# manish-pra/sampling-gpmpc

Hardware: AMD Instinct MI355X
Metric: sampled trajectory-steps/sec (Ns*H per wall second) (higher is better)
Workload: dtype f64; 1 GPU; BASELINE configs[1]: params_pendulum1D_samples, sequential re-conditioned rollout (mode R, value+gradient labels T=3), Ns=1024 per GPU, H=30; Ns_per_gpu=1024, H=30, Ns_total=1024, device=AMD Radeon Graphics (gfx950:sramecc+:xnack-), cus=256

## Files before the change

sampling_gpmpc_amd/csrc/build.py:

```python
#!/usr/bin/env python3
import hashlib
import json
import os
import subprocess
import sys
from concurrent.futures import ThreadPoolExecutor

HERE = os.path.dirname(os.path.abspath(__file__))
REPO = os.path.dirname(os.path.dirname(HERE))
SOURCES = ["capi.hip", "rollout.hip", "rollout_fast.hip", "rollout_tiles.hip", "rollout_one.hip", "rollout_indep.hip", "joint.hip",
           "joint_mfma.hip", "joint_chol.hip", "assemble.hip", "base_samples.hip", "hull.hip",
           "hull_query.hip", "sup_dev.hip", "mll.hip", "moments.hip", "moments_grad.hip", "tube_qp.hip", "tube_rows.hip", "pathwise.hip",
           "pathwise_stats.hip", "pathwise_grad.hip", "pathwise_cand.hip", "robust_tube.hip", "robust_tube_grad.hip", "lipschitz.hip", "contraction.hip",
           "optimistic.hip"]
HEADERS = ["gpmpc_device.hpp", "gpmpc_host.hpp", "rollout_args.hpp", "rollout_plan.hpp", "joint_args.hpp", "joint_eigh.hpp", "joint_plan.hpp", "hull_geom.hpp", "min_index.hpp", "base_stream.hpp", "moments_step.hpp", "pathwise_step.hpp", "robust_step.hpp", "contraction_math.hpp",
           "rollout_one_gen.inc", "rollout_tiles_mfma.inc", "joint_mfma_gen.inc",
           os.path.join(REPO, "include", "gpmpc_hip.h")]
GENERATED = {"rollout_one_gen.inc": os.path.join(REPO, "tools", "gen_rollout_one.py"),
             "rollout_tiles_mfma.inc": os.path.join(REPO, "tools", "gen_mfma_chains.py"),
             "joint_mfma_gen.inc": os.path.join(REPO, "tools", "gen_joint_mfma.py")}
OUT = os.path.join(os.path.dirname(HERE), "libgpmpc_hip.so")
OBJDIR = os.path.join(HERE, "build")
HIPCC = os.environ.get("HIPCC", "/opt/rocm/bin/hipcc")
FLAGS = ["--offload-arch=gfx950", "-O3", "-std=c++17", "-fPIC", "-fgpu-rdc" if False else "-fno-gpu-rdc",
         "-ffp-contract=on", "-I", os.path.join(REPO, "include"), "-I", HERE]
FLAGS += os.environ.get("GPMPC_EXTRA_DEFS", "").split()
if os.environ.get("GPMPC_PHASE_TIMERS") == "1":
    FLAGS.append("-DGPMPC_PHASE_TIMERS")


EXTRA_FLAGS = {"rollout_fast.hip": os.environ.get("GPMPC_FAST_FLAGS", "-mllvm -disable-machine-licm").split(),
               "joint.hip": os.environ.get("GPMPC_JOINT_FLAGS", "-mllvm -disable-machine-licm").split(),
               "rollout.hip": os.environ.get("GPMPC_ROLLOUT_FLAGS", "-mllvm -disable-machine-licm").split(),
               "rollout_tiles.hip": os.environ.get("GPMPC_TILES_FLAGS", "").split(),
               "rollout_one.hip": os.environ.get("GPMPC_ONE_FLAGS", "-mllvm -disable-machine-licm -mllvm -amdgpu-load-store-vectorizer=0").split(),
               "rollout_indep.hip": os.environ.get("GPMPC_INDEP_FLAGS", "").split(),
               "joint_mfma.hip": os.environ.get("GPMPC_JOINT_MFMA_FLAGS", "").split(),
               "pathwise_stats.hip": os.environ.get("GPMPC_PATHWISE_STATS_FLAGS", "-mllvm -disable-machine-licm").split(),
               "pathwise_grad.hip": os.environ.get("GPMPC_PATHWISE_GRAD_FLAGS", "-mllvm -disable-machine-licm").split(),
               "pathwise_cand.hip": os.environ.get("GPMPC_PATHWISE_CAND_FLAGS", "-mllvm -disable-machine-licm").split()}


STAMP = os.path.join(OBJDIR, "flags.stamp")


def _mtime(p):
    return os.path.getmtime(p) if os.path.exists(p) else 0.0


def flags_digest():
    blob = json.dumps({"hipcc": HIPCC, "flags": FLAGS, "extra": EXTRA_FLAGS}, sort_keys=True)
    return hashlib.sha256(blob.encode()).hexdigest()


def is_default_build():
    return not (os.environ.get("GPMPC_EXTRA_DEFS") or os.environ.get("GPMPC_PHASE_TIMERS") == "1"
                or os.environ.get("GPMPC_FAST_FLAGS") is not None)


def clean_objdir():
    if not os.path.isdir(OBJDIR):
        return
    for name in os.listdir(OBJDIR):
        p = os.path.join(OBJDIR, name)
        if os.path.isfile(p) and not (name.endswith(".o") and "-hip-amdgcn" not in name) and name != "flags.stamp":
            os.remove(p)


def build(force=False, verbose=False):
    os.makedirs(OBJDIR, exist_ok=True)
    clean_objdir()
    digest = flags_digest()
    try:
        with open(STAMP) as f:
            stale_flags = f.read().strip() != digest
    except OSError:
        stale_flags = True
    force = force or stale_flags
    hdr_t = max(_mtime(h if os.path.isabs(h) else os.path.join(HERE, h)) for h in HEADERS)
    hdr_t = max(hdr_t, _mtime(os.path.abspath(__file__)))
    jobs = []
    for src in SOURCES:
        s = os.path.join(HERE, src)
        o = os.path.join(OBJDIR, src.replace(".hip", ".o"))
        if force or _mtime(o) < max(_mtime(s), hdr_t):
            jobs.append((s, o))
    def cc(job):
        s, o = job
        cmd = [HIPCC, "-x", "hip", "-c", s, "-o", o] + FLAGS + EXTRA_FLAGS.get(os.path.basename(s), [])
        if verbose:
            print(" ".join(cmd), flush=True)
        r = subprocess.run(cmd, capture_output=True, text=True)
        if r.returncode != 0:
            raise RuntimeError(f"hipcc failed for {s}:\n{r.stdout}\n{r.stderr}")
        if verbose and r.stderr.strip():
            print(r.stderr)
    with ThreadPoolExecutor(max_workers=4) as ex:
        list(ex.map(cc, jobs))
    with open(STAMP, "w") as f:
        f.write(digest + "\n")
    objs = [os.path.join(OBJDIR, s.replace(".hip", ".o")) for s in SOURCES]
    if jobs or not os.path.exists(OUT):
        cmd = [HIPCC, "-shared", "-fPIC", "--offload-arch=gfx950", "-o", OUT] + objs
        if verbose:
            print(" ".join(cmd), flush=True)
        r = subprocess.run(cmd, capture_output=True, text=True)
        if r.returncode != 0:
            raise RuntimeError(f"link failed:\n{r.stdout}\n{r.stderr}")
    return OUT


if __name__ == "__main__":
    out = build(force="--force" in sys.argv, verbose="--verbose" in sys.argv or "-v" in sys.argv)
    print(out)
```

sampling_gpmpc_amd/csrc/rollout.hip:

```cpp
#include "gpmpc_host.hpp"
#include "rollout_plan.hpp"

#include <algorithm>

namespace gpmpc {


__device__ long long g_phase_cycles[16];
#define GPMPC_PHASE(idx)                                                  \
    do {                                                                  \
        const long long _now = __builtin_readcyclecounter();              \
        ph[idx] += _now - tph;                                            \
        tph = _now;                                                       \
    } while (0)

__device__ __forceinline__ void wave_lds_sync() {
    __builtin_amdgcn_fence(__ATOMIC_ACQ_REL, "wavefront");
    __builtin_amdgcn_wave_barrier();
}


template <int T, int RPL, bool FAC_LDS>
__global__ __launch_bounds__(64 * GPMPC_MAX_NY) void rollout_kernel(const RolloutArgs a) {
    constexpr int D = 2;
// ... 408 lines not shown
    g.lds_bytes = ((size_t)g.lds_shared + (size_t)s.g_ny * g.lds_per_wave) * sizeof(double);
    if (g.lds_bytes > (size_t)(160 * 1024 - 256)) {
        g.status = GPMPC_E_UNSUPPORTED;
        g.msg = "rollout: horizon too long for LDS vectors";
    }
    g.grid = s.Ns;
    g.block = 64 * s.g_ny;
    if (s.mode == GPMPC_MODE_RECONDITIONED && !g.fac_lds && !s.state)
        g.ws_bytes = (size_t)s.Ns * s.g_ny * g.ws_chain_stride * sizeof(double);
    return g;
}

template <int T, int RPL>
static int launch_rollout(const RolloutArgs& args, const RolloutLaunch& p, hipStream_t stream) {
    const dim3 grid((unsigned)p.grid), block(p.block);
    if (p.fac_lds) {
        auto k = rollout_kernel<T, RPL, true>;
        GPMPC_HIP_CHECK(hipFuncSetAttribute((const void*)k, hipFuncAttributeMaxDynamicSharedMemorySize, (int)p.lds_bytes));
        hipLaunchKernelGGL(k, grid, block, p.lds_bytes, stream, args);
    } else {
        auto k = rollout_kernel<T, RPL, false>;
        GPMPC_HIP_CHECK(hipFuncSetAttribute((const void*)k, hipFuncAttributeMaxDynamicSharedMemorySize, (int)p.lds_bytes));
        hipLaunchKernelGGL(k, grid, block, p.lds_bytes, stream, args);
    }
    GPMPC_HIP_CHECK(hipGetLastError());
    return GPMPC_OK;
}

int rollout_generic_launch(const RolloutArgs& args, const RolloutLaunch& p, hipStream_t st) {
    if (p.T == 1) {
        if (p.rpl == 1) return launch_rollout<1, 1>(args, p, st);
        if (p.rpl == 2) return launch_rollout<1, 2>(args, p, st);
        return launch_rollout<1, 4>(args, p, st);
    } else if (p.T == 3) {
        if (p.rpl == 1) return launch_rollout<3, 1>(args, p, st);
        if (p.rpl == 2) return launch_rollout<3, 2>(args, p, st);
        return launch_rollout<3, 4>(args, p, st);
    }
    return fail(GPMPC_E_UNSUPPORTED, "rollout: only T = 1 and T = 3 (D = 2) are instantiated");
}

static int g_rollout_pin = GPMPC_KERNEL_AUTO;

static int knob(const char* name) {
    const char* e = std::getenv(name);
    return !e ? 0 : (e[0] == '1' ? 1 : (e[0] == '0' ? -1 : 0));
}

static RolloutKnobs rollout_knobs() {
    RolloutKnobs k;
    k.pin = g_rollout_pin;
    k.one = knob("GPMPC_ROLLOUT_ONE");
    k.tiles = knob("GPMPC_ROLLOUT_TILES");
    k.disable_fast = knob("GPMPC_DISABLE_FAST_ROLLOUT") > 0;
    k.disable_grid_root = knob("GPMPC_DISABLE_GRID_ROOT") > 0;
    k.force_global_factor = knob("GPMPC_FORCE_GLOBAL_FACTOR") > 0;
    return k;
}

static RolloutShape rollout_shape(const gpmpc_gp_desc_t* gp, const gpmpc_env_desc_t* env, int mode, int hall_tasks, int64_t Ns, int H,
                                  int n_h0 = 0, int n_v0 = 0, bool state = false, int state_slots = 0, int state_points = 0) {
    return RolloutShape{gp->T, gp->D, gp->N_r, observed_real_slots(gp), gp->real_has_grad, gp->g_ny, gp->grid_n0, gp->grid_n1,
                        env ? env->env_id : -1, env ? env->nx : GPMPC_MAX_NX, mode, (mode == GPMPC_MODE_INDEPENDENT) ? gp->T : hall_tasks,
                        Ns, H, n_h0, n_v0, state, state ? state_slots : 0, state_points};
}

}

using namespace gpmpc;

extern "C" {

static int g_last_rollout_path = -1;
int gpmpc_debug_last_rollout_path(void) { return g_last_rollout_path; }
int gpmpc_rollout_last_kernel(void) { return g_last_rollout_path; }
int gpmpc_rollout_kernel_for(const gpmpc_gp_desc_t* gp, const gpmpc_env_desc_t* env, int32_t mode, int32_t hall_tasks, int64_t Ns,
                             int32_t H) {
    if (check_gp(gp) != GPMPC_OK || check_env(gp, env) != GPMPC_OK) return GPMPC_KERNEL_AUTO;
    return plan_rollout_launch(rollout_shape(gp, env, mode, hall_tasks, Ns, H), rollout_knobs()).kernel;
}
int gpmpc_rollout_pin_kernel(int32_t kernel) {
    const int prev = gpmpc::g_rollout_pin;
    gpmpc::g_rollout_pin = (kernel >= GPMPC_KERNEL_GENERIC && kernel <= GPMPC_KERNEL_ONE) ? kernel : GPMPC_KERNEL_AUTO;
    return prev;
}

int gpmpc_debug_rollout_plan(const gpmpc_gp_desc_t* gp, const gpmpc_env_desc_t* env, int32_t mode, int32_t hall_tasks, int64_t Ns,
                             int32_t H, int32_t n_h0, int32_t n_v0, int32_t state_slots, int32_t state_points, char* out, size_t out_len) {
    if (int rc = check_gp(gp)) return rc;
    if (int rc = check_env(gp, env)) return rc;
    if (!out || out_len < 1 || Ns < 1 || H < 1 || n_h0 < 0 || n_v0 < 0 || state_slots < 0)
        return fail(GPMPC_E_ARG, "gpmpc_debug_rollout_plan: bad arguments");
    const RolloutLaunch p = plan_rollout_launch(
        rollout_shape(gp, env, mode, hall_tasks, Ns, H, n_h0, n_v0, state_slots > 0, state_slots, state_points), rollout_knobs());
    const char* env_name = (p.env_id == GPMPC_ENV_PENDULUM1D) ? "pendulum" : "car";
    char k[128];
    if (p.status != GPMPC_OK) {
        snprintf(out, out_len, "error=%d %s", p.status, p.msg);
        return GPMPC_OK;
    }
    switch (p.kernel) {
        case GPMPC_KERNEL_ONE: snprintf(k, sizeof k, "rollout_one_kernel<N0=4,ENV=pendulum>"); break;
        case GPMPC_KERNEL_TILES:
            snprintf(k, sizeof k, "rollout_tiles_kernel<N0=%d,N1=9,ENV=%s,NT=%d,SEED=%d>", p.n0, env_name, p.nt, p.seed);
            break;
        case GPMPC_KERNEL_FAST:
// ... 155 lines not shown
```

sampling_gpmpc_amd/csrc/rollout_one.hip:

```cpp
#include "gpmpc_host.hpp"
#include "rollout_plan.hpp"

#include <type_traits>
#include <utility>

namespace gpmpc {

#include "rollout_one_gen.inc"

__device__ long long g_one_phase_cycles[16];
__device__ double g_one_dbg[64 * 64];

#ifdef GPMPC_PHASE_TIMERS
#define OPH_DECL long long oph_[10] = {0, 0, 0, 0, 0, 0, 0, 0, 0, 0}; long long opht_ = __builtin_readcyclecounter()
#define OPH(i) do { const long long n_ = __builtin_readcyclecounter(); oph_[i] += n_ - opht_; opht_ = n_; } while (0)
#define OPH_T(i) OPH(i)
#define OPH_STORE do { if (blockIdx.x == 0 && threadIdx.x == 0) { for (int i_ = 0; i_ < 8; ++i_) g_one_phase_cycles[i_] = oph_[i_]; g_one_phase_cycles[10] = oph_[8]; g_one_phase_cycles[11] = oph_[9]; } } while (0)
#elif defined(GPMPC_ONE_PHASE_MARKS)
#define OPH_DECL
#define OPH(i) asm volatile("; one_phase_end " #i)
#define OPH_T(i)
#define OPH_STORE
#else
#define OPH_DECL
#define OPH(i)
#define OPH_T(i)
#define OPH_STORE
#endif
#ifdef GPMPC_ONE_PHASE_MARKS
#define OPH_MARK(name) asm volatile("; one_phase_" name)
#else
#define OPH_MARK(name)
#endif
#ifndef GPMPC_ONE_DEBUG_STEP
#define GPMPC_ONE_DEBUG_STEP 2
#endif
#ifndef GPMPC_ONE_DEBUG_ROW
#define GPMPC_ONE_DEBUG_ROW 0
#endif
#ifdef GPMPC_ONE_DEBUG
#define ODBG(slot, val) do { if (blockIdx.x == 0 && t == GPMPC_ONE_DEBUG_STEP) g_one_dbg[(slot) * 64 + lane] = (val); } while (0)
#else
#define ODBG(slot, val)
#endif

constexpr int kOneMaxRows = 4 * kOneNTR;
constexpr int kOneRS = 5;

__device__ __forceinline__ void one_sync_lds() {
    __builtin_amdgcn_fence(__ATOMIC_ACQ_REL, "wavefront");
    __builtin_amdgcn_wave_barrier();
}
template <int B, int E, class F>
__device__ __forceinline__ void one_for(F&& f) {
    if constexpr (B < E) {
        f(std::integral_constant<int, B>{});
        one_for<B + 1, E>(f);
    }
}
template <int B, int E, class F>
__device__ __forceinline__ void one_pick_row(int v, F&& f) {
    if constexpr (E - B == 1) {
        f(std::integral_constant<int, B>{});
    } else if constexpr (E - B > 1) {
        constexpr int M = (B + E) / 2;
        if (v < M) one_pick_row<B, M>(v, f);
        else one_pick_row<M, E>(v, f);
    }
}
__device__ __forceinline__ double one_mfma_zero(double a, double b) {
    double d;
    asm volatile("s_nop 1\n\tv_mfma_f64_4x4x4_4b_f64 %0, %1, %2, 0\n\ts_nop 5" : "=&v"(d) : "v"(a), "v"(b));
    return d;
}
template <int CTRL>
__device__ __forceinline__ double one_add_rot(double v) {
    const int lo = __builtin_amdgcn_mov_dpp(__double2loint(v), CTRL, 0xf, 0xf, true);
    const int hi = __builtin_amdgcn_mov_dpp(__double2hiint(v), CTRL, 0xf, 0xf, true);
    return v + __hiloint2double(hi, lo);
}
__device__ __forceinline__ double one_block_sum(double v) { return one_add_rot<0x124>(one_add_rot<0x128>(v)); }
template <int BQ>
__device__ __forceinline__ double one_merge(double dst, double w) {
    const int lo = __builtin_amdgcn_update_dpp(__double2loint(dst), __double2loint(w), 0xe4, 0xf, 1 << BQ, false);
    const int hi = __builtin_amdgcn_update_dpp(__double2hiint(dst), __double2hiint(w), 0xe4, 0xf, 1 << BQ, false);
    return __hiloint2double(hi, lo);
}
__device__ __forceinline__ double one_bpermute(double v, int addr) {
    const int lo = __builtin_amdgcn_ds_bpermute(addr, __double2loint(v));
    const int hi = __builtin_amdgcn_ds_bpermute(addr, __double2hiint(v));
    return __hiloint2double(hi, lo);
}
__device__ __forceinline__ void one_min3(double& m, double a, double b, double c) {
    asm("v_min_f64 %0, %0, %1\n\tv_min_f64 %0, %0, %2\n\tv_min_f64 %0, %0, %3" : "+v"(m) : "v"(a), "v"(b), "v"(c));
// ... 182 lines not shown
                                              double (&invB)[3], bool& okA, bool& okB, double& ex) {
    double s10[2] = {A[1][0], B[1][0]}, s20[2] = {A[2][0], B[2][0]}, s21[2] = {A[2][1], B[2][1]};
    double s11[2] = {A[1][1], B[1][1]}, s22[2] = {A[2][2], B[2][2]};
    double d1[2], d2[2], y1[2], y2[2], h[2], t[2], e[2], l10[2], l20[2], l21[2], n21[2], p2[2], r1[2], r2[2];
    double n, r, rr, a0, a1, a2, a4;
    int ni;
    GPMPC_ONE_FENCE();
    GPMPC_ONE_LVL(l10[m_] = s10[m_] * p.y0[m_]; l20[m_] = s20[m_] * p.y0[m_], n = x * k.log2e);
    GPMPC_ONE_LVL(d1[m_] = fma(-l10[m_], l10[m_], s11[m_]); n21[m_] = fma(-l20[m_], l10[m_], s21[m_]), n = rint(n));
    GPMPC_ONE_LVL(y1[m_] = __builtin_amdgcn_rsq(d1[m_]); h[m_] = 0.5 * d1[m_]; p2[m_] = fma(-l20[m_], l20[m_], s22[m_]),
                  r = fma(n, k.nln2h, x));
    GPMPC_ONE_LVL(t[m_] = h[m_] * y1[m_], r = fma(n, k.nln2l, r); ni = (int)n);
    GPMPC_ONE_LVL(e[m_] = fma(-t[m_], y1[m_], 0.5), rr = r * r; a0 = 1.0 + r; a1 = fma(k.c3, r, k.c2));
    GPMPC_ONE_LVL(y1[m_] = fma(y1[m_], e[m_], y1[m_]), a0 = fma(a1, rr, a0); a4 = fma(k.c9, r, k.c8); a1 = fma(k.c11, r, k.c10));
    GPMPC_ONE_LVL(l21[m_] = n21[m_] * y1[m_]; r1[m_] = d1[m_] * y1[m_], a4 = fma(a1, rr, a4); a2 = fma(k.c5, r, k.c4));
    GPMPC_ONE_LVL(d2[m_] = fma(-l21[m_], l21[m_], p2[m_]), a1 = fma(k.c7, r, k.c6));
    GPMPC_ONE_LVL(y2[m_] = __builtin_amdgcn_rsq(d2[m_]); h[m_] = 0.5 * d2[m_], a2 = fma(a1, rr, a2); rr = rr * rr);
    GPMPC_ONE_LVL(t[m_] = h[m_] * y2[m_], a2 = fma(a4, rr, a2));
    GPMPC_ONE_LVL(e[m_] = fma(-t[m_], y2[m_], 0.5), a0 = fma(a2, rr, a0));
    GPMPC_ONE_LVL(y2[m_] = fma(y2[m_], e[m_], y2[m_]), ex = ldexp(a0, ni));
    GPMPC_ONE_LVL(r2[m_] = d2[m_] * y2[m_], (void)0);
    asm volatile("" ::"v"(p.r0[0]), "v"(r1[0]), "v"(r2[0]), "v"(p.r0[1]), "v"(r1[1]), "v"(r2[1]));
    okA = (p.d0[0] > 0.0) && (d1[0] > 0.0) && (d2[0] > 0.0);
    okB = (p.d0[1] > 0.0) && (d1[1] > 0.0) && (d2[1] > 0.0);
    LA[0][0] = p.r0[0], LA[1][0] = l10[0], LA[2][0] = l20[0], LA[1][1] = r1[0], LA[2][1] = l21[0], LA[2][2] = r2[0];
    LB[0][0] = p.r0[1], LB[1][0] = l10[1], LB[2][0] = l20[1], LB[1][1] = r1[1], LB[2][1] = l21[1], LB[2][2] = r2[1];
    LA[0][1] = LA[0][2] = LA[1][2] = 0.0;
    LB[0][1] = LB[0][2] = LB[1][2] = 0.0;
    invA[0] = p.y0[0], invA[1] = y1[0], invA[2] = y2[0];
    invB[0] = p.y0[1], invB[1] = y1[1], invB[2] = y2[1];
}

typedef const __attribute__((address_space(4))) RolloutArgs* OneArgsPtr;
typedef __attribute__((address_space(3))) double* OneLdsRow;
__device__ __forceinline__ OneArgsPtr one_cold_args(OneArgsPtr p) {
    asm volatile("" : "+s"(p));
    return p;
}
__device__ __forceinline__ long one_cold_sample(int s) {
    asm volatile("" : "+s"(s));
    return s;
}

__device__ __forceinline__ bool one_wanted(double* p) {
    asm volatile("" : "+s"(p));
    return p != nullptr;
}
struct OneLds {
    static constexpr int VR = 0;
    static constexpr int HS = ((4 * kOneNKT * kOneRS + 1) & ~1);
    static constexpr int TOTAL = HS + 96 * kOneRS;
};

template <int N0, int ENV, bool LEAN>
__global__ __launch_bounds__(64, 1) void rollout_one_kernel(const RolloutArgs a) {
    static_assert(ENV == GPMPC_ENV_PENDULUM1D && N0 == 4, "instantiated for the pendulum1D 4 x 9 grid");
    constexpr int D = 2, T = 3, N1 = 9, NR = N0 * N1, NX = 2;
    constexpr int NKT = kOneNKT;
    constexpr int KFIRST = NKT >> 2, KLAST = (NKT + kOneNTR - 1) >> 2;
    static_assert(4 * NKT == NR && N0 + N1 <= 16, "panel map generated for N_r = 36");
    extern __shared__ __attribute__((aligned(16))) double smem[];
#ifdef GPMPC_PHASE_TIMERS
    const long long opk0_ = __builtin_readcyclecounter();
#endif

    const GpParams& gp = a.gp;
    const OneArgsPtr ak0 = (OneArgsPtr)__builtin_amdgcn_kernarg_segment_ptr();
    const int s32 = blockIdx.x;
    const int lane = threadIdx.x;
    const int kq = lane >> 4, bm = (lane >> 2) & 3, jq = lane & 3;
    const long s = blockIdx.x;
    const int H = a.H;
    double* VRb = smem + OneLds::VR;
    double* HSb = smem + OneLds::HS;

    const double il0 = gp.inv_l2[0][0], il1 = gp.inv_l2[0][1], os = gp.os[0];
    const int lr = (lane < NR) ? lane : 0, ga = lr / N1, gc = lr - ga * N1;
    double qa[N0], qb[N1];
#pragma unroll
    for (int j = 0; j < N0; ++j) qa[j] = plan_grid_Qa(a.plan, gp, 0)[j * N0 + ga];
#pragma unroll
    for (int j = 0; j < N1; ++j) qb[j] = plan_grid_Qb(a.plan, gp, 0)[j * N1 + gc];
    double dsc_ld = plan_grid_dsc(a.plan, gp, 0)[lr], w_ld = plan_grid_w(a.plan, gp, 0)[lr];
    const bool g_ax0 = lane < N0;
    const int g_pt = g_ax0 ? lane * N1 : ((lane < N0 + N1) ? lane - N0 : 0);
    const bool g_axis = lane < N0 + N1, g_sel0 = g_ax0 || !g_axis;
    double g_x = a.X_r[g_pt * D + (g_ax0 ? 0 : 1)];
    const double il0_lane = g_axis ? (g_ax0 ? il0 : il1) : il0, il1_lane = g_axis ? 0.0 : il1;
    const int bp_addr = (lane & 15) << 2;
    constexpr int kPt0 = N0 + N1;
    const int jpt = lane - kPt0;
    const double Inat = (kq == jq) ? 1.0 : 0.0;
    const double MK[4] = {(bm == 0) ? 1.0 : 0.0, (bm == 1) ? 1.0 : 0.0, (bm == 2) ? 1.0 : 0.0, (bm == 3) ? 1.0 : 0.0};
    const int vr_rd = (4 * bm + kq) * kOneRS + jq;
    const int hs_rd = (4 * (bm - NKT) + kq) * kOneRS + jq;
    unsigned hs_wr = (unsigned)(size_t)(OneLdsRow)(HSb + 3 * jpt * kOneRS), vr_wr = (unsigned)(size_t)(OneLdsRow)(VRb + lane * kOneRS);
    asm volatile("" : "+v"(hs_wr), "+v"(vr_wr));
    const int rA = 4 * bm + jq;

    double x[NX];
#pragma unroll
    for (int d = 0; d < NX; ++d) x[d] = a.x0[(a.x0_per_sample ? s * NX : 0) + d];
    double xq[NX] = {0.0, 0.0};
    double zq[T], uq;
    const int lz = (lane < H) ? lane : 0;
#pragma unroll
    for (int c = 0; c < T; ++c) zq[c] = a.z[(long)lz * a.z_step_stride + s * T + c];
    uq = a.u_ff[lz];
// ... 82 lines not shown
        constexpr int nh = decltype(nhc)::value;
        constexpr int i0 = nh & 3, ycol = (i0 + 3) & 3;
        constexpr int cb0 = i0, cb1 = (i0 + 1) & 3, cb2 = (i0 + 2) & 3;
        const unsigned ha = hs_wr, va = vr_wr;
        double vr4[4];
        vr4[cb0] = e.vr[0], vr4[cb1] = e.vr[1], vr4[cb2] = e.vr[2], vr4[ycol] = w_lane;
        if constexpr (nh > 0) {
            double h4[T][4];
#pragma unroll
            for (int aa = 0; aa < T; ++aa)
                h4[aa][cb0] = e.hs[aa][0], h4[aa][cb1] = e.hs[aa][1], h4[aa][cb2] = e.hs[aa][2], h4[aa][ycol] = yt[aa];
            asm volatile("s_mov_b32 exec_lo, 0xffffe000\n\ts_mov_b32 exec_hi, 0x1fff\n\t"
                         "ds_write2_b64 %[ha], %[a0], %[a1] offset1:1\n\t"
                         "ds_write2_b64 %[ha], %[a2], %[a3] offset0:2 offset1:3\n\t"
                         "ds_write2_b64 %[ha], %[b0], %[b1] offset0:5 offset1:6\n\t"
                         "ds_write2_b64 %[ha], %[b2], %[b3] offset0:7 offset1:8\n\t"
                         "ds_write2_b64 %[ha], %[c0], %[c1] offset0:10 offset1:11\n\t"
                         "ds_write2_b64 %[ha], %[c2], %[c3] offset0:12 offset1:13\n\t"
                         "s_mov_b32 exec_lo, -1\n\ts_mov_b32 exec_hi, 0xf\n\t"
                         "ds_write2_b64 %[va], %[v0], %[v1] offset1:1\n\t"
                         "ds_write2_b64 %[va], %[v2], %[v3] offset0:2 offset1:3\n\t"
                         "s_mov_b64 exec, -1"
                         :
                         : [ha] "v"(ha), [va] "v"(va), [a0] "v"(h4[0][0]), [a1] "v"(h4[0][1]), [a2] "v"(h4[0][2]), [a3] "v"(h4[0][3]),
                           [b0] "v"(h4[1][0]), [b1] "v"(h4[1][1]), [b2] "v"(h4[1][2]), [b3] "v"(h4[1][3]), [c0] "v"(h4[2][0]),
                           [c1] "v"(h4[2][1]), [c2] "v"(h4[2][2]), [c3] "v"(h4[2][3]), [v0] "v"(vr4[0]), [v1] "v"(vr4[1]), [v2] "v"(vr4[2]),
                           [v3] "v"(vr4[3])
                         : "memory");
        } else {
            asm volatile("s_mov_b32 exec_lo, -1\n\ts_mov_b32 exec_hi, 0xf\n\t"
                         "ds_write2_b64 %[va], %[v0], %[v1] offset1:1\n\t"
                         "ds_write2_b64 %[va], %[v2], %[v3] offset0:2 offset1:3\n\t"
                         "s_mov_b64 exec, -1"
                         :
                         : [va] "v"(va), [v0] "v"(vr4[0]), [v1] "v"(vr4[1]), [v2] "v"(vr4[2]), [v3] "v"(vr4[3])
                         : "memory");
        }
    };

    double ucur;
    {
        double kk, Rq0, Rq1;
        const double ea = one_exp_neg(ent_a(0, true, x, ucur), ek);
        ent_b(0, ea, x[0], ucur, kk, Rq0, Rq1);
        OneEntC e;
        ent_c_vals(false, kk, x[0], ucur, Rq0, Rq1, e);
        ent_c_put(std::integral_constant<int, 0>{}, e);
    }
#ifdef GPMPC_PHASE_TIMERS
    opht_ = __builtin_readcyclecounter();
#endif
    OPH_MARK("end prologue");

    auto step = [&](auto Kc) {
        constexpr int K = decltype(Kc)::value;
        constexpr int R0 = 4 * K - NKT;
        const int i0 = n_h & 3, ycol = (i0 + 3) & 3, npts = t;
        const int cb0 = i0, cb1 = (i0 + 1) & 3, cb2 = (i0 + 2) & 3;
        const bool more = t + 1 < H;
        one_sync_lds();
        double Vu[K + 1], RN[K + 1];
        Vu[0] = VRb[vr_rd];
        Vu[1] = VRb[vr_rd + 16 * kOneRS];
        double t8 = VRb[(32 + kq) * kOneRS + jq];
#pragma unroll
        for (int g = KFIRST; g <= K; ++g) RN[g] = HSb[max(hs_rd + 16 * g * kOneRS, 0)];
        asm volatile("" : "+v"(t8), "+v"(RN[K]));
        Vu[2] = (bm == 0) ? t8 : 0.0;
#pragma unroll
        for (int g = 3; g <= K; ++g) Vu[g] = 0.0;
        OPH(0);

        double S0, S1;
        one_solve<K>(P, Vu, RN, MK, n_h, S0, S1, ud, drow, dcol, Inat);
        ODBG(0, Vu[0]);
        ODBG(1, Vu[1]);
        ODBG(2, Vu[2]);
        if constexpr (K >= 3) ODBG(3, Vu[3]);
        ODBG(5, RN[2]);
        OPH(2);

        double mu[T], S[T][T], zt[T];
        const double Stot = one_block_sum(S0 + S1);
        ODBG(6, Stot);
        const int cb[T] = {cb0, cb1, cb2};
        auto extract = [&](auto bc) {
            constexpr int bq = decltype(bc)::value;
#pragma unroll
            for (int c = 0; c <= bq; ++c) {
                const double kss = (bq == c) ? ((bq == 0) ? os : ((bq == 1) ? os * il0 : os * il1)) : 0.0;
                const double val = kss - readlane_f64(Stot, 16 * cb[bq] + cb[c]);
                S[bq][c] = val;
                S[c][bq] = val;
            }
        };
        auto var = [&](int bq) { return fmax(S[bq][bq], gp.var_floor); };
        auto fetch = [&](auto bc) {
            constexpr int bq = decltype(bc)::value;
            mu[bq] = readlane_f64(Stot, 16 * cb[bq] + ycol);
            zt[bq] = readlane_f64(zq[bq], t);
        };
        extract(std::integral_constant<int, 0>{});
        fetch(std::integral_constant<int, 0>{});
        OPH(3);
        OneCholPair ch;
        one_chol_pivot1(S[0][0] + gp.noise[0], S[0][0], ch);
        double y0s;
        {
            double acc = 0.0;
            acc = fma(ch.r0[1], zt[0], acc);
            y0s = acc + mu[0];
        }
        double x0n, un, kk, Rq0, Rq1;
        x0n = x[0] + x[1] * a.env.dt;
        {
            const bool mine = jpt == npts;
            xh[0] = mine ? x[0] : xh[0];
            xh[1] = mine ? ucur : xh[1];
        }
        double earg;
        {
            const double xs[NX] = {x0n, x[1] + y0s};
            earg = ent_a(t + 1, more, xs, un);
        }
        extract(std::integral_constant<int, 1>{});
        extract(std::integral_constant<int, 2>{});
        one_min3(s_min, S[0][0], S[1][1], S[2][2]);
        bool all_zero = false;
        if (!LEAN && a.var_zero_thr >= 0.0) all_zero = (var(0) <= a.var_zero_thr) && (var(1) <= a.var_zero_thr) && (var(2) <= a.var_zero_thr);
        double Rt[T][T], C[T][T], cinv[T];
        bool c_ok, r_ok;
        {
            double Sn[T][T], rinv[T], ea;
#pragma unroll
            for (int bq = 0; bq < T; ++bq)
#pragma unroll
                for (int c = 0; c < T; ++c) Sn[bq][c] = S[bq][c] + ((bq == c) ? gp.noise[bq] : 0.0);
            one_chol_rest(Sn, S, ch, earg, ek, C, Rt, cinv, rinv, c_ok, r_ok, ea);
            ent_b(t + 1, ea, x0n, un, kk, Rq0, Rq1);
        }
        fetch(std::integral_constant<int, 1>{});
        fetch(std::integral_constant<int, 2>{});
        double y[T];
        bool clip;
        auto draw = [&]() {
            clip = false;
#pragma unroll
            for (int bq = 0; bq < T; ++bq) {
                double acc = 0.0;
#pragma unroll
                for (int c = 0; c <= bq; ++c) acc = fma(Rt[bq][c], zt[c], acc);
                const double yb = acc + mu[bq];
                const double dlt = yb - mu[bq];
                clip = clip || (dlt * dlt > a.beta * a.beta * S[bq][bq]);
                y[bq] = yb;
            }
        };
        if (__builtin_expect(!r_ok, 0)) info_acc |= root_small_fast_retry<T>(S, one_cold_args(ak0)->gp.jitter, Rt);
        draw();
        if (__builtin_expect(clip || all_zero || !r_ok, 0)) {
            OPH_MARK("cold begin");
            if (all_zero) {
#pragma unroll
                for (int bq = 0; bq < T; ++bq) y[bq] = mu[bq];
                clip = false;
            }
            if (clip) {
#pragma unroll
                for (int bq = 0; bq < T; ++bq) {
                    const double dlt = y[bq] - mu[bq];
                    if (dlt * dlt > a.beta * a.beta * var(bq)) {
                        const double sd = a.beta * sqrt(var(bq));
                        y[bq] = fmin(fmax(y[bq], mu[bq] - sd), mu[bq] + sd);
                    }
                }
            }
            if (y[0] != y0s) {
                const double xs[NX] = {x0n, x[1] + y[0]};
                const double ea = one_exp_neg(ent_a(t + 1, more, xs, un), ek);
                ent_b(t + 1, ea, x0n, un, kk, Rq0, Rq1);
            }
            OPH_MARK("cold end");
        }
        if (!LEAN && lane == 0 && one_wanted(Y_s)) {
#pragma unroll
            for (int bq = 0; bq < T; ++bq) Y_s[t * T + bq] = y[bq];
        }
        OPH(4);

        if (more) {
            if (!c_ok) info_acc |= GPMPC_INFO_TRAIN_CHOL_FAIL;
            {
                const bool mine = jpt == npts;
#pragma unroll
                for (int bq = 0; bq < T; ++bq) yt[bq] = mine ? y[bq] : yt[bq];
            }
            OneEntC ec;
            ent_c_vals(true, kk, x0n, un, Rq0, Rq1, ec);
            const double sv[OV_COUNT] = {0.0, C[0][0], C[1][0], C[1][1], C[2][0], C[2][1], C[2][2], cinv[0], cinv[1], cinv[2], Vu[K]};
            auto inverse_tiles = [&](double U, double dr, double dcl) -> double {
                const double M = Inat - dr * U;
                const double Mt = one_mfma_zero(M, Inat);
                const double M2 = one_mfma_zero(Mt, M);
                const double Pq = one_mfma_zero(Inat + Mt, Inat + M2);
                return Pq * dcl;
            };
            constexpr bool INV_IN_SOLVE = K >= kOneSolveInvK;
            constexpr int TB = OneEpoch<K>::t_begin, TE = OneEpoch<K>::t_end < kOneAppendSteps ? OneEpoch<K>::t_end : kOneAppendSteps;
            one_pick_row<TB, TE>(t, [&](auto tc) {
                constexpr int TT = decltype(tc)::value, NH = T * TT;
                constexpr int i0 = NH & 3;
                constexpr int tn = NH >> 2;
                constexpr int bt = (NKT + tn) & 3;
                constexpr int lo = NH - 4 * R0;
                static_assert(((NKT + tn) >> 2) == K && lo == 4 * bt + i0 && tn >= 0 && tn < kOneNTR, "step outside its epoch");
#ifdef GPMPC_ONE_DEBUG
                if (n_h != NH) g_one_dbg[63 * 64 + lane] = (double)(n_h - NH);
#endif
                ent_c_put(std::integral_constant<int, NH + T>{}, ec);
                OPH(1);
                one_hset_row_at<tn, NH>(Vu);
                if constexpr (i0 >= 2 && tn + 1 < kOneNTR) {
                    double Vm[K + 2];
#pragma unroll
                    for (int gg = 0; gg <= K; ++gg) Vm[gg] = Vu[gg];
                    Vm[K + 1] = 0.0;
                    Vm[K] = one_apply<OnePatReach<i0, bt>>(Vu[K], sv);
                    one_hset_row_at<tn + 1, NH>(Vm);
                }
                OPH(5);
                ud = one_apply<OnePatDiag<lo>>(ud, sv);
                drow = one_apply<OnePatInvRow<lo>>(drow, sv);
                dcol = one_apply<OnePatInvCol<lo>>(dcol, sv);
                OPH_T(9);
                if constexpr (K < KLAST && lo + 3 > 16) {
                    ud1 = one_apply<OnePatDiag<lo - 16>>(ud1, sv);
                    drow1 = one_apply<OnePatInvRow<lo - 16>>(drow1, sv);
                    dcol1 = one_apply<OnePatInvCol<lo - 16>>(dcol1, sv);
                    const double G1 = inverse_tiles(ud1, drow1, dcol1);
                    one_hset_gd<K + 1>(G1);
                }
                if constexpr (INV_IN_SOLVE && TT == OneEpoch<K>::t_end - 1) one_hset_gd<K>(inverse_tiles(ud, drow, dcol));
            });
            one_for<(R0 > 0 ? R0 : 0), (R0 + 5 < kOneNTR ? R0 + 5 : kOneNTR)>([&](auto rc) { one_touch_row<decltype(rc)::value>(P); });
            if constexpr (K < KLAST) one_touch_gd<K + 1>(P);
            OPH_T(8);
            if constexpr (INV_IN_SOLVE) {
                one_touch_gd<K>(P);
            } else {
                const double Gt = inverse_tiles(ud, drow, dcol);
                ODBG(8, ud);
                ODBG(9, Gt);
                one_put_gd<K>(P, Gt);
            }
            n_h += T;
        }
        OPH(6);

        x[1] = x[1] + y[0];
        x[0] = x0n;
        ucur = un;
        t += 1;
        OPH(7);
    };

    one_for<KFIRST, KLAST + 1>([&](auto Kc) {
        constexpr int K = decltype(Kc)::value;
#pragma unroll 1
        while (t < H && t < OneEpoch<K>::t_end) step(Kc);
        ud = ud1, drow = drow1, dcol = dcol1;
        ud1 = Inat, drow1 = 1.0, dcol1 = 1.0;
    });

    if (s_min < gp.var_floor) info_acc |= GPMPC_INFO_VAR_CLAMPED;
    {
        const OneArgsPtr ak = one_cold_args(ak0);
        const long se = one_cold_sample(s32);
        double* const X_traj = ak->X_traj;
        if (lane <= H) {
#pragma unroll
            for (int d = 0; d < NX; ++d) X_traj[(se * NX + d) * (H + 1) + lane] = (lane == H) ? x[d] : xq[d];
        }
        if (lane == 0) ak->info[se] = info_acc;
    }
    OPH_STORE;
#ifdef GPMPC_PHASE_TIMERS
    if (blockIdx.x == 0 && threadIdx.x == 0) g_one_phase_cycles[9] = __builtin_readcyclecounter() - opk0_;
#endif
}

RolloutLaunch rollout_one_sizing(const RolloutShape& s, const RolloutLaunch& g) {
    RolloutLaunch p = g;
    p.kernel = GPMPC_KERNEL_AUTO;
    if (s.mode != GPMPC_MODE_RECONDITIONED || s.T != 3 || s.D != 2 || s.hall_tasks != 3 || s.real_has_grad) return p;
    if (!plan_has_grid_root(s.grid_n0, s.grid_n1, s.real_has_grad)) return p;
    if (s.env_id != GPMPC_ENV_PENDULUM1D || s.g_ny != 1 || s.grid_n0 != 4 || s.grid_n1 != 9) return p;
    if (s.H < 2 || 3 * (s.H - 1) > kOneMaxRows) return p;
    p.kernel = GPMPC_KERNEL_ONE;
    p.grid = s.Ns;
    p.block = 64;
    p.lds_bytes = (size_t)OneLds::TOTAL * sizeof(double);
    p.ws_bytes = 0;
    return p;
}

int rollout_one_launch(const RolloutArgs& args, const RolloutLaunch& p, hipStream_t st) {
    const bool lean = args.Y == nullptr && args.Xi == nullptr && !(args.var_zero_thr >= 0.0);
    auto k = lean ? rollout_one_kernel<4, GPMPC_ENV_PENDULUM1D, true> : rollout_one_kernel<4, GPMPC_ENV_PENDULUM1D, false>;
    GPMPC_HIP_CHECK(hipFuncSetAttribute((const void*)k, hipFuncAttributeMaxDynamicSharedMemorySize, (int)p.lds_bytes));
    hipLaunchKernelGGL(k, dim3((unsigned)p.grid), dim3(p.block), p.lds_bytes, st, args);
    GPMPC_HIP_CHECK(hipGetLastError());
    return GPMPC_OK;
}

}

extern "C" int gpmpc_debug_read_one_phases(long long* out ) {
    GPMPC_HIP_CHECK(hipMemcpyFromSymbol(out, HIP_SYMBOL(gpmpc::g_one_phase_cycles), 16 * sizeof(long long)));
    return GPMPC_OK;
}
extern "C" int gpmpc_debug_read_one(double* out ) {
    GPMPC_HIP_CHECK(hipMemcpyFromSymbol(out, HIP_SYMBOL(gpmpc::g_one_dbg), 64 * 64 * sizeof(double)));
    return GPMPC_OK;
}
```

sampling_gpmpc_amd/csrc/rollout_plan.hpp:

```cpp
#pragma once
#include "gpmpc_host.hpp"
#include "rollout_args.hpp"

namespace gpmpc {

struct RolloutShape {
    int T, D, N_r, n_r, real_has_grad;
    int g_ny, grid_n0, grid_n1;
    int env_id, nx;
    int mode, hall_tasks;
    long Ns;
    int H, n_h0, n_v0;
    int state;
    int state_slots, state_points;
};

struct RolloutKnobs {
    int pin;
    int one, tiles;
    int disable_fast, disable_grid_root, force_global_factor;
};

struct RolloutLaunch {
    int status;
    const char* msg;
    int kernel;
    int T, rpl, fac_lds;
    int env_id, lhh_lds, grid_root;
    int n0, nt, seed;
    long grid;
    int block;
    size_t lds_bytes;
    size_t ws_bytes;
    size_t zero_bytes;
    int nh_max, lds_shared, lds_per_wave, linv_in_lds, max_points;
    long ws_chain_stride;
};

RolloutLaunch rollout_generic_sizing(const RolloutShape& s, bool force_global);
RolloutLaunch rollout_fast_sizing(const RolloutShape& s, const RolloutLaunch& g, bool grid_root, bool force_global);
RolloutLaunch rollout_tiles_sizing(const RolloutShape& s, const RolloutLaunch& g);
RolloutLaunch rollout_one_sizing(const RolloutShape& s, const RolloutLaunch& g);
RolloutLaunch rollout_indep_sizing(const RolloutShape& s, const RolloutLaunch& g, bool grid_root);

int rollout_generic_launch(const RolloutArgs& args, const RolloutLaunch& p, hipStream_t st);
int rollout_fast_launch(const RolloutArgs& args, const RolloutLaunch& p, hipStream_t st);
int rollout_tiles_launch(const RolloutArgs& args, const RolloutLaunch& p, hipStream_t st);
int rollout_one_launch(const RolloutArgs& args, const RolloutLaunch& p, hipStream_t st);
int rollout_indep_launch(const RolloutArgs& args, const RolloutLaunch& p, hipStream_t st);

inline RolloutLaunch plan_rollout_launch(const RolloutShape& s, const RolloutKnobs& k) {
    const RolloutLaunch g = rollout_generic_sizing(s, k.force_global_factor);
    const RolloutLaunch one = rollout_one_sizing(s, g), tiles = rollout_tiles_sizing(s, g);
    const RolloutLaunch fast = rollout_fast_sizing(s, g, !k.disable_grid_root, k.force_global_factor);
    const RolloutLaunch indep = rollout_indep_sizing(s, g, !k.disable_grid_root);
    const long chains = s.Ns * s.g_ny;
    const bool seeded = s.n_h0 > 0 || s.n_v0 > 0 || s.state;
    const bool pinned = k.pin != GPMPC_KERNEL_AUTO;
    const int one_md = pinned ? (k.pin == GPMPC_KERNEL_ONE ? 1 : -1) : k.one;
    const int tiles_md = pinned ? (k.pin == GPMPC_KERNEL_TILES ? 1 : -1) : k.tiles;
    const bool use_fast = (pinned ? k.pin == GPMPC_KERNEL_FAST : !k.disable_fast) && fast.kernel == GPMPC_KERNEL_FAST;
    const bool use_one = one_md >= 0 && !k.disable_fast && !k.disable_grid_root && !k.force_global_factor &&
                         !(one_md == 0 && k.tiles > 0) && one.kernel == GPMPC_KERNEL_ONE && (one_md > 0 || s.Ns <= 2048);
    const bool tuned_alt = !seeded && use_fast;
    const bool use_tiles = tiles_md >= 0 && !k.disable_fast && !k.disable_grid_root && tiles.kernel == GPMPC_KERNEL_TILES &&
                           (tiles_md > 0 || (tuned_alt ? chains > (s.g_ny == 1 ? 1024 : 768) : chains >= 256));
    const bool use_indep = k.pin != GPMPC_KERNEL_GENERIC && !k.disable_fast && indep.kernel == GPMPC_KERNEL_INDEP;
    if (seeded) return (!s.state && use_tiles) ? tiles : g;
    return use_one ? one : use_tiles ? tiles : use_fast ? fast : use_indep ? indep : g;
}

}
```

Before: 497.9 million trajectory-steps/s.

## Fully unroll rollout_one time steps with compile-time step indices

Adds a STEPS variant of the single-wave rollout kernel that recursively instantiates every horizon step with a compile-time index, replacing the runtime step loop, row picker and counters with per-step specialized code and a generated per-step solve. The last step finishes and ends the program inline, and retry handling moves into the cold path. It is made the default for the lean launch, which aims to cut loop overhead and runtime indexing. The cost is a much larger code footprint, with risk of instruction-cache pressure and longer compile times.

```diff
diff --git a/sampling_gpmpc_amd/csrc/build.py b/sampling_gpmpc_amd/csrc/build.py
--- a/sampling_gpmpc_amd/csrc/build.py
+++ b/sampling_gpmpc_amd/csrc/build.py
@@ -14,11 +14,12 @@
            "pathwise_stats.hip", "pathwise_grad.hip", "pathwise_cand.hip", "robust_tube.hip", "robust_tube_grad.hip", "lipschitz.hip", "contraction.hip",
            "optimistic.hip"]
 HEADERS = ["gpmpc_device.hpp", "gpmpc_host.hpp", "rollout_args.hpp", "rollout_plan.hpp", "joint_args.hpp", "joint_eigh.hpp", "joint_plan.hpp", "hull_geom.hpp", "min_index.hpp", "base_stream.hpp", "moments_step.hpp", "pathwise_step.hpp", "robust_step.hpp", "contraction_math.hpp",
-           "rollout_one_gen.inc", "rollout_tiles_mfma.inc", "joint_mfma_gen.inc",
+           "rollout_one_gen.inc", "rollout_one_steps_gen.inc", "rollout_tiles_mfma.inc", "joint_mfma_gen.inc",
            os.path.join(REPO, "include", "gpmpc_hip.h")]
 GENERATED = {"rollout_one_gen.inc": os.path.join(REPO, "tools", "gen_rollout_one.py"),
              "rollout_tiles_mfma.inc": os.path.join(REPO, "tools", "gen_mfma_chains.py"),
              "joint_mfma_gen.inc": os.path.join(REPO, "tools", "gen_joint_mfma.py")}
+BUILD_GENERATED = {"rollout_one_steps_gen.inc": (os.path.join(REPO, "tools", "gen_rollout_one.py"), "--steps-out")}
 OUT = os.path.join(os.path.dirname(HERE), "libgpmpc_hip.so")
 OBJDIR = os.path.join(HERE, "build")
 HIPCC = os.environ.get("HIPCC", "/opt/rocm/bin/hipcc")
@@ -67,7 +68,22 @@
             os.remove(p)
 
 
+def generate():
+    for inc, (gen, flag) in BUILD_GENERATED.items():
+        out = os.path.join(HERE, inc)
+        if _mtime(out) < _mtime(gen):
+            tmp = out + f".{os.getpid()}.tmp"
+            r = subprocess.run([sys.executable, gen, flag, tmp], capture_output=True, text=True)
+            if r.returncode != 0:
+                raise RuntimeError(f"{os.path.basename(gen)} {flag} failed:\n{r.stdout}\n{r.stderr}")
+            os.replace(tmp, out)
+
+
+generate()
+
+
 def build(force=False, verbose=False):
+    generate()
     os.makedirs(OBJDIR, exist_ok=True)
     clean_objdir()
     digest = flags_digest()
diff --git a/sampling_gpmpc_amd/csrc/rollout.hip b/sampling_gpmpc_amd/csrc/rollout.hip
--- a/sampling_gpmpc_amd/csrc/rollout.hip
+++ b/sampling_gpmpc_amd/csrc/rollout.hip
@@ -484,6 +484,7 @@
     k.pin = g_rollout_pin;
     k.one = knob("GPMPC_ROLLOUT_ONE");
     k.tiles = knob("GPMPC_ROLLOUT_TILES");
+    k.one_steps = knob("GPMPC_ROLLOUT_ONE_STEPS");
     k.disable_fast = knob("GPMPC_DISABLE_FAST_ROLLOUT") > 0;
     k.disable_grid_root = knob("GPMPC_DISABLE_GRID_ROOT") > 0;
     k.force_global_factor = knob("GPMPC_FORCE_GLOBAL_FACTOR") > 0;
diff --git a/sampling_gpmpc_amd/csrc/rollout_one.hip b/sampling_gpmpc_amd/csrc/rollout_one.hip
--- a/sampling_gpmpc_amd/csrc/rollout_one.hip
+++ b/sampling_gpmpc_amd/csrc/rollout_one.hip
@@ -7,6 +7,7 @@
 namespace gpmpc {
 
 #include "rollout_one_gen.inc"
+#include "rollout_one_steps_gen.inc"
 
 __device__ long long g_one_phase_cycles[16];
 __device__ double g_one_dbg[64 * 64];
@@ -32,6 +33,11 @@
 #else
 #define OPH_MARK(name)
 #endif
+#ifdef GPMPC_ONE_PHASE_MARKS
+#define OPH_STEP(ts) asm volatile("; one_steps_head %0" : : "n"(ts))
+#else
+#define OPH_STEP(ts)
+#endif
 #ifndef GPMPC_ONE_DEBUG_STEP
 #define GPMPC_ONE_DEBUG_STEP 2
 #endif
@@ -39,7 +45,7 @@
 #define GPMPC_ONE_DEBUG_ROW 0
 #endif
 #ifdef GPMPC_ONE_DEBUG
-#define ODBG(slot, val) do { if (blockIdx.x == 0 && t == GPMPC_ONE_DEBUG_STEP) g_one_dbg[(slot) * 64 + lane] = (val); } while (0)
+#define ODBG(slot, val) do { if (blockIdx.x == 0 && tl == GPMPC_ONE_DEBUG_STEP) g_one_dbg[(slot) * 64 + lane] = (val); } while (0)
 #else
 #define ODBG(slot, val)
 #endif
@@ -328,8 +334,9 @@
     static constexpr int TOTAL = HS + 96 * kOneRS;
 };
 
-template <int N0, int ENV, bool LEAN>
-__global__ __launch_bounds__(64, 1) void rollout_one_kernel(const RolloutArgs a) {
+constexpr int one_epoch_of(int t) { return (kOneNKT + ((3 * t) >> 2)) >> 2; }
+template <int N0, int ENV, bool LEAN, bool STEPS>
+__device__ __forceinline__ void rollout_one_body(const RolloutArgs& a) {
     static_assert(ENV == GPMPC_ENV_PENDULUM1D && N0 == 4, "instantiated for the pendulum1D 4 x 9 grid");
     constexpr int D = 2, T = 3, N1 = 9, NR = N0 * N1, NX = 2;
     constexpr int NKT = kOneNKT;
@@ -518,12 +525,36 @@
 #endif
     OPH_MARK("end prologue");
 
-    auto step = [&](auto Kc) {
+    auto finish = [&](double xe0, double xe1) __attribute__((always_inline)) {
+        const double xe[NX] = {xe0, xe1};
+        if (s_min < gp.var_floor) info_acc |= GPMPC_INFO_VAR_CLAMPED;
+        {
+            const OneArgsPtr ak = one_cold_args(ak0);
+            const long se = one_cold_sample(s32);
+            double* const X_traj = ak->X_traj;
+            if (lane <= H) {
+#pragma unroll
+                for (int d = 0; d < NX; ++d) X_traj[(se * NX + d) * (H + 1) + lane] = (lane == H) ? xe[d] : xq[d];
+            }
+            if (lane == 0) ak->info[se] = info_acc;
+        }
+        OPH_STORE;
+#ifdef GPMPC_PHASE_TIMERS
+        if (blockIdx.x == 0 && threadIdx.x == 0) g_one_phase_cycles[9] = __builtin_readcyclecounter() - opk0_;
+#endif
+    };
+
+    auto step = [&](auto Kc, auto TSc, auto&& next) {
         constexpr int K = decltype(Kc)::value;
+        constexpr int TS = decltype(TSc)::value;
+        constexpr bool ST = TS >= 0;
+        static_assert(!ST || (one_epoch_of(TS) == K && TS >= OneEpoch<K>::t_begin && TS < OneEpoch<K>::t_end), "step outside its epoch");
         constexpr int R0 = 4 * K - NKT;
-        const int i0 = n_h & 3, ycol = (i0 + 3) & 3, npts = t;
+        const int tl = ST ? TS : t, nhl = ST ? T * TS : n_h;
+        const int i0 = nhl & 3, ycol = (i0 + 3) & 3, npts = tl;
         const int cb0 = i0, cb1 = (i0 + 1) & 3, cb2 = (i0 + 2) & 3;
-        const bool more = t + 1 < H;
+        const bool more = (ST && TS >= kOneAppendSteps) ? false : tl + 1 < H;
+        if constexpr (ST) OPH_STEP(TS);
         one_sync_lds();
         double Vu[K + 1], RN[K + 1];
         Vu[0] = VRb[vr_rd];
@@ -538,7 +569,8 @@
         OPH(0);
 
         double S0, S1;
-        one_solve<K>(P, Vu, RN, MK, n_h, S0, S1, ud, drow, dcol, Inat);
+        if constexpr (ST) one_solve_t<TS>(P, Vu, RN, MK, S0, S1, ud, drow, dcol, Inat);
+        else one_solve<K>(P, Vu, RN, MK, n_h, S0, S1, ud, drow, dcol, Inat);
         ODBG(0, Vu[0]);
         ODBG(1, Vu[1]);
         ODBG(2, Vu[2]);
@@ -564,7 +596,7 @@
         auto fetch = [&](auto bc) {
             constexpr int bq = decltype(bc)::value;
             mu[bq] = readlane_f64(Stot, 16 * cb[bq] + ycol);
-            zt[bq] = readlane_f64(zq[bq], t);
+            zt[bq] = readlane_f64(zq[bq], tl);
         };
         extract(std::integral_constant<int, 0>{});
         fetch(std::integral_constant<int, 0>{});
@@ -587,7 +619,7 @@
         double earg;
         {
             const double xs[NX] = {x0n, x[1] + y0s};
-            earg = ent_a(t + 1, more, xs, un);
+            earg = ent_a(tl + 1, more, xs, un);
         }
         extract(std::integral_constant<int, 1>{});
         extract(std::integral_constant<int, 2>{});
@@ -603,7 +635,7 @@
 #pragma unroll
                 for (int c = 0; c < T; ++c) Sn[bq][c] = S[bq][c] + ((bq == c) ? gp.noise[bq] : 0.0);
             one_chol_rest(Sn, S, ch, earg, ek, C, Rt, cinv, rinv, c_ok, r_ok, ea);
-            ent_b(t + 1, ea, x0n, un, kk, Rq0, Rq1);
+            ent_b(tl + 1, ea, x0n, un, kk, Rq0, Rq1);
         }
         fetch(std::integral_constant<int, 1>{});
         fetch(std::integral_constant<int, 2>{});
@@ -622,9 +654,7 @@
                 y[bq] = yb;
             }
         };
-        if (__builtin_expect(!r_ok, 0)) info_acc |= root_small_fast_retry<T>(S, one_cold_args(ak0)->gp.jitter, Rt);
-        draw();
-        if (__builtin_expect(clip || all_zero || !r_ok, 0)) {
+        auto cold = [&]() __attribute__((always_inline)) {
             OPH_MARK("cold begin");
             if (all_zero) {
 #pragma unroll
@@ -643,18 +673,42 @@
             }
             if (y[0] != y0s) {
                 const double xs[NX] = {x0n, x[1] + y[0]};
-                const double ea = one_exp_neg(ent_a(t + 1, more, xs, un), ek);
-                ent_b(t + 1, ea, x0n, un, kk, Rq0, Rq1);
+                const double ea = one_exp_neg(ent_a(tl + 1, more, xs, un), ek);
+                ent_b(tl + 1, ea, x0n, un, kk, Rq0, Rq1);
             }
             OPH_MARK("cold end");
+        };
+        if constexpr (!ST) {
+            if (__builtin_expect(!r_ok, 0)) info_acc |= root_small_fast_retry<T>(S, one_cold_args(ak0)->gp.jitter, Rt);
+            draw();
+            if (__builtin_expect(clip || all_zero || !r_ok, 0)) cold();
+        } else {
+            draw();
+            if (__builtin_expect(clip || all_zero || !r_ok || !more, 0)) {
+                if (!r_ok) {
+                    info_acc |= root_small_fast_retry<T>(S, one_cold_args(ak0)->gp.jitter, Rt);
+                    draw();
+                }
+                if (clip || all_zero || !r_ok) cold();
+                if (!more) {
+                    finish(x0n, x[1] + y[0]);
+                    asm volatile("s_endpgm" : : : "memory");
+                }
+            }
         }
         if (!LEAN && lane == 0 && one_wanted(Y_s)) {
 #pragma unroll
-            for (int bq = 0; bq < T; ++bq) Y_s[t * T + bq] = y[bq];
+            for (int bq = 0; bq < T; ++bq) Y_s[tl * T + bq] = y[bq];
         }
         OPH(4);
 
-        if (more) {
+        auto handover = [&]() __attribute__((always_inline)) {
+            x[1] = x[1] + y[0];
+            x[0] = x0n;
+            ucur = un;
+        };
+        if constexpr (!ST || TS < kOneAppendSteps)
+        if (ST || more) {
             if (!c_ok) info_acc |= GPMPC_INFO_TRAIN_CHOL_FAIL;
             {
                 const bool mine = jpt == npts;
@@ -673,7 +727,7 @@
             };
             constexpr bool INV_IN_SOLVE = K >= kOneSolveInvK;
             constexpr int TB = OneEpoch<K>::t_begin, TE = OneEpoch<K>::t_end < kOneAppendSteps ? OneEpoch<K>::t_end : kOneAppendSteps;
-            one_pick_row<TB, TE>(t, [&](auto tc) {
+            auto block = [&](auto tc) {
                 constexpr int TT = decltype(tc)::value, NH = T * TT;
                 constexpr int i0 = NH & 3;
                 constexpr int tn = NH >> 2;
@@ -681,7 +735,7 @@
                 constexpr int lo = NH - 4 * R0;
                 static_assert(((NKT + tn) >> 2) == K && lo == 4 * bt + i0 && tn >= 0 && tn < kOneNTR, "step outside its epoch");
 #ifdef GPMPC_ONE_DEBUG
-                if (n_h != NH) g_one_dbg[63 * 64 + lane] = (double)(n_h - NH);
+                if (nhl != NH) g_one_dbg[63 * 64 + lane] = (double)(nhl - NH);
 #endif
                 ent_c_put(std::integral_constant<int, NH + T>{}, ec);
                 OPH(1);
@@ -707,7 +761,9 @@
                     one_hset_gd<K + 1>(G1);
                 }
                 if constexpr (INV_IN_SOLVE && TT == OneEpoch<K>::t_end - 1) one_hset_gd<K>(inverse_tiles(ud, drow, dcol));
-            });
+            };
+            if constexpr (!ST) one_pick_row<TB, TE>(t, block);
+            else if constexpr (TS < kOneAppendSteps) block(TSc);
             one_for<(R0 > 0 ? R0 : 0), (R0 + 5 < kOneNTR ? R0 + 5 : kOneNTR)>([&](auto rc) { one_touch_row<decltype(rc)::value>(P); });
             if constexpr (K < KLAST) one_touch_gd<K + 1>(P);
             OPH_T(8);
@@ -719,41 +775,53 @@
                 ODBG(9, Gt);
                 one_put_gd<K>(P, Gt);
             }
-            n_h += T;
+            if constexpr (!ST) n_h += T;
         }
         OPH(6);
-
-        x[1] = x[1] + y[0];
-        x[0] = x0n;
-        ucur = un;
-        t += 1;
+        handover();
+        if constexpr (!ST) t += 1;
         OPH(7);
+        if constexpr (ST) next();
     };
 
-    one_for<KFIRST, KLAST + 1>([&](auto Kc) {
-        constexpr int K = decltype(Kc)::value;
+    if constexpr (!STEPS) {
+        one_for<KFIRST, KLAST + 1>([&](auto Kc) {
+            constexpr int K = decltype(Kc)::value;
 #pragma unroll 1
-        while (t < H && t < OneEpoch<K>::t_end) step(Kc);
-        ud = ud1, drow = drow1, dcol = dcol1;
-        ud1 = Inat, drow1 = 1.0, dcol1 = 1.0;
-    });
-
-    if (s_min < gp.var_floor) info_acc |= GPMPC_INFO_VAR_CLAMPED;
-    {
-        const OneArgsPtr ak = one_cold_args(ak0);
-        const long se = one_cold_sample(s32);
-        double* const X_traj = ak->X_traj;
-        if (lane <= H) {
-#pragma unroll
-            for (int d = 0; d < NX; ++d) X_traj[(se * NX + d) * (H + 1) + lane] = (lane == H) ? x[d] : xq[d];
-        }
-        if (lane == 0) ak->info[se] = info_acc;
-    }
-    OPH_STORE;
-#ifdef GPMPC_PHASE_TIMERS
-    if (blockIdx.x == 0 && threadIdx.x == 0) g_one_phase_cycles[9] = __builtin_readcyclecounter() - opk0_;
-#endif
-}
+            while (t < H && t < OneEpoch<K>::t_end) step(Kc, std::integral_constant<int, -1>{}, [] {});
+            ud = ud1, drow = drow1, dcol = dcol1;
+            ud1 = Inat, drow1 = 1.0, dcol1 = 1.0;
+        });
+    } else {
+        auto run = [&](auto& self, auto tc) __attribute__((always_inline)) -> void {
+            constexpr int TS = decltype(tc)::value, K = one_epoch_of(TS);
+            step(std::integral_constant<int, K>{}, tc, [&]() __attribute__((always_inline)) {
+                if constexpr (TS < kOneAppendSteps) {
+                    if constexpr (TS + 1 == OneEpoch<K>::t_end) {
+                        ud = ud1, drow = drow1, dcol = dcol1;
+                        ud1 = Inat, drow1 = 1.0, dcol1 = 1.0;
+                    }
+                    self(self, std::integral_constant<int, TS + 1>{});
+                }
+            });
+        };
+        run(run, std::integral_constant<int, 0>{});
+    }
+
+    if constexpr (!STEPS) finish(x[0], x[1]);
+}
+
+template <int N0, int ENV, bool LEAN>
+__global__ __launch_bounds__(64, 1) void rollout_one_kernel(const RolloutArgs a) {
+    rollout_one_body<N0, ENV, LEAN, false>(a);
+}
+template <int N0, int ENV>
+__global__ __launch_bounds__(64, 1) void rollout_one_steps_kernel(const RolloutArgs a) {
+    rollout_one_body<N0, ENV, true, true>(a);
+}
+
+constexpr bool kOneStepsDefault = true;
+static int g_one_last_form = -1;
 
 RolloutLaunch rollout_one_sizing(const RolloutShape& s, const RolloutLaunch& g) {
     RolloutLaunch p = g;
@@ -772,7 +840,10 @@
 
 int rollout_one_launch(const RolloutArgs& args, const RolloutLaunch& p, hipStream_t st) {
     const bool lean = args.Y == nullptr && args.Xi == nullptr && !(args.var_zero_thr >= 0.0);
-    auto k = lean ? rollout_one_kernel<4, GPMPC_ENV_PENDULUM1D, true> : rollout_one_kernel<4, GPMPC_ENV_PENDULUM1D, false>;
+    const bool steps = lean && (p.one_steps != 0 ? p.one_steps > 0 : kOneStepsDefault);
+    auto k = steps ? rollout_one_steps_kernel<4, GPMPC_ENV_PENDULUM1D>
+                   : (lean ? rollout_one_kernel<4, GPMPC_ENV_PENDULUM1D, true> : rollout_one_kernel<4, GPMPC_ENV_PENDULUM1D, false>);
+    g_one_last_form = steps ? 1 : 0;
     GPMPC_HIP_CHECK(hipFuncSetAttribute((const void*)k, hipFuncAttributeMaxDynamicSharedMemorySize, (int)p.lds_bytes));
     hipLaunchKernelGGL(k, dim3((unsigned)p.grid), dim3(p.block), p.lds_bytes, st, args);
     GPMPC_HIP_CHECK(hipGetLastError());
@@ -781,6 +852,7 @@
 
 }
 
+extern "C" int gpmpc_debug_last_rollout_one_form(void) { return gpmpc::g_one_last_form; }
 extern "C" int gpmpc_debug_read_one_phases(long long* out ) {
     GPMPC_HIP_CHECK(hipMemcpyFromSymbol(out, HIP_SYMBOL(gpmpc::g_one_phase_cycles), 16 * sizeof(long long)));
     return GPMPC_OK;
diff --git a/sampling_gpmpc_amd/csrc/rollout_plan.hpp b/sampling_gpmpc_amd/csrc/rollout_plan.hpp
--- a/sampling_gpmpc_amd/csrc/rollout_plan.hpp
+++ b/sampling_gpmpc_amd/csrc/rollout_plan.hpp
@@ -19,6 +19,7 @@
     int pin;
     int one, tiles;
     int disable_fast, disable_grid_root, force_global_factor;
+    int one_steps = 0;
 };
 
 struct RolloutLaunch {
@@ -28,6 +29,7 @@
     int T, rpl, fac_lds;
     int env_id, lhh_lds, grid_root;
     int n0, nt, seed;
+    int one_steps;
     long grid;
     int block;
     size_t lds_bytes;
@@ -67,7 +69,12 @@
                            (tiles_md > 0 || (tuned_alt ? chains > (s.g_ny == 1 ? 1024 : 768) : chains >= 256));
     const bool use_indep = k.pin != GPMPC_KERNEL_GENERIC && !k.disable_fast && indep.kernel == GPMPC_KERNEL_INDEP;
     if (seeded) return (!s.state && use_tiles) ? tiles : g;
-    return use_one ? one : use_tiles ? tiles : use_fast ? fast : use_indep ? indep : g;
+    if (use_one) {
+        RolloutLaunch p = one;
+        p.one_steps = k.one_steps;
+        return p;
+    }
+    return use_tiles ? tiles : use_fast ? fast : use_indep ? indep : g;
 }
 
 }
```

After: 539.5 million trajectory-steps/s, median of 6. 1.08x the previous value.
